# SonghuaHu-UMD/MultiSTGraph

Hardware: AMD Instinct MI355X
Metric: forward node-steps/s (B*T*N per second), MultiATGCN.predict (higher is better)
Workload: dtype f32; 1 GPU; Baltimore 403-node, in=24h out=24h, batch=64/GPU, multi+unidirection K=5; nodes=403, per_gpu_batch=64, global_batch=64, in_steps=24, out_steps=24, parallelism=batch shards, no data-path collective (dp1), layer_wavefront_streams=True

## Files before the change

multistgraph_amd/csrc/matgcn_capi.hip:

```cpp
#include <hip/hip_runtime.h>
#include <stdint.h>
#include <stdio.h>
#include <stdlib.h>
#include <string.h>

#include "../../include/matgcn.h"
#include "matgcn_internal.h"

#include "matgcn_kernels.hip"
#include "matgcn_node16.hip"
#include "matgcn_bwd_kernels.hip"
#include "matgcn_mc_scores.hip"
#include "matgcn_conformal.hip"
#include "matgcn_regions.hip"
#include "matgcn_optim.hip"
#include "matgcn_loss.hip"
#include "matgcn_region_loss.hip"
#include "matgcn_crps.hip"
#include "matgcn_head_mc_bwd.hip"

namespace {

constexpr int H = 64;
constexpr int MAX_STEPS = 64;
// ... 927 lines not shown
      CHECK_LAUNCH();
      if (multi && l + 1 < P.L) HIP_OK(hipEventRecord(W.step[l][t], cs));
      return MATGCN_OK;
    }
    if (l > 0 && t == nextChunk[l]) {
      const int nt = chunk_steps(P, t);
      nextChunk[l] = t + nt;
      float* slot; long stride;
      int mixedSteps = 0;
      if (shared_mix_slot(c, l - 1, t, &slot, &stride)) mixedSteps = P.T - 1 - t < nt ? P.T - 1 - t : nt;
      if (multi) {
        if (mixedSteps == nt) HIP_OK(hipStreamWaitEvent(xs, W.mixed[l - 1][t + nt], 0));
        else HIP_OK(hipStreamWaitEvent(xs, W.step[l - 1][t + nt - 1], 0));
      }
      RETURN_IF(hoist_x(c, l, below + t * stepRows, t, nt, xs, mixedSteps));
      if (multi) {
        HIP_OK(hipEventRecord(W.xdone[l][t], xs));
        HIP_OK(hipStreamWaitEvent(cs, W.xdone[l][t], 0));
      }
    }
    Node16Args res;
    if (l == 0)
      fill_res_args(c, l, x0p + (long)t * P.Np * P.C0, (long)P.T * P.Np * P.C0,
                    c.prm->weights_gru + (size_t)l * P.T + t, seq + t * stepRows, &res);
    else
      fill_res_args(c, l, below + t * stepRows, (long)P.Np * H, c.prm->weights_gru + (size_t)l * P.T + t,
                    seq + t * stepRows, &res);
    const bool zs = zeroStart && t == 0;
    if (!zs) RETURN_IF(cell_phase(c, l, t, 0, nullptr, &res, cs));
    if (multi && l + 1 < P.L) HIP_OK(hipEventRecord(W.mixed[l][t], cs));
    if (lazyPrep && multi && l == 0 && t == 0) RETURN_IF(prep_wait(cs, 1));
    RETURN_IF(cell_phase(c, l, t, 1, nullptr, &res, cs, zs));
    if (!zs) RETURN_IF(cell_phase(c, l, t, 2, nullptr, &res, cs));
    RETURN_IF(cell_phase(c, l, t, 3, nullptr, &res, cs, zs));
    if (multi && l + 1 < P.L) HIP_OK(hipEventRecord(W.step[l][t], cs));
    return MATGCN_OK;
  };
  for (int l = 0; l < P.L; ++l)
    for (int t = 0; t < P.T; ++t) RETURN_IF(enqueue_step(l, t));
  for (int l = 0; l < P.L; ++l) {
    hipStream_t cs = chain_stream(l);
    if (finalsUser) {
      hipLaunchKernelGGL(k_unpack_rows, dim3(blocks_for((size_t)P.B * P.N * H)), dim3(256), 0, cs, c.ws + P.oHx[l],
                         finalsUser + (size_t)l * P.B * P.N * H, P.B, P.N, P.Np, H);
      CHECK_LAUNCH();
    }
    if (multi && l > 0) HIP_OK(hipEventRecord(W.done[l], cs));
  }
  if (multi)
    for (int l = 1; l < P.L; ++l) HIP_OK(hipStreamWaitEvent(c.s, W.done[l], 0));
  return MATGCN_OK;
}

int encoder_padded(const Ctx& c, const float* x0p, const float* h0User, float* finalsUser) {
  const int rc = encoder_chains(c, x0p, h0User, finalsUser);
  if (rc != MATGCN_OK) join_library_streams(c.s);
  return rc;
}

int fuse_padded(const Ctx& c, const float* X, float* x0p, const int32_t* labelStart = nullptr,
                const int32_t* relSteps = nullptr, int64_t seriesSteps = 0) {
  const Plan& P = c.P;
  const matgcn_dims* D = c.D;
  FuseArgs a;
  memset(&a, 0, sizeof(a));
  a.X = X; a.x0 = x0p; a.tsg = c.prm->weight_tsg;
  a.labelStart = labelStart; a.seriesSteps = (long)seriesSteps;
  if (labelStart)
    for (int s2 = 0; s2 < D->x_steps; ++s2) a.rel[s2] = relSteps[s2];
  for (int h = 0; h < D->n_heads; ++h) { a.ts[h] = c.prm->weight_ts[h]; a.headBegin[h] = D->head_begin[h]; }
  for (int j = 0; j < P.C0 - P.od; ++j) a.extSrc[j] = D->ext_src[j];
  a.B = P.B; a.T = P.T; a.N = P.N; a.Np = P.Np; a.C0 = P.C0; a.od = P.od; a.F = D->x_feat;
  a.xSteps = D->x_steps; a.startDim = D->start_dim; a.nHeads = D->n_heads; a.nTs = D->n_ts;
  hipLaunchKernelGGL(k_fuse_heads, dim3(blocks_for((size_t)P.B * P.T * P.Np)), dim3(256), 0, c.s, a);
  return launch_ok();
}

int head_padded(const Ctx& c, const float* seqp, float* out) {
  const Plan& P = c.P;
  HeadArgs a;
  a.seq = seqp + (size_t)(P.T - P.headT) * P.B * P.Np * H; a.w = c.prep + P.oHead;
  a.bias = c.prm->end_conv_bias; a.out = out;
  a.B = P.B; a.T = P.headT; a.N = P.N; a.Np = P.Np; a.CH = P.CH; a.od = P.od; a.NTc = P.NTc;
  ProfScope prof(MATGCN_PROF_HEAD, c.s);
  hipLaunchKernelGGL(k_head, dim3((unsigned)(P.B * ((P.N + 31) / 32))), dim3(256), 0, c.s, a);
  return launch_ok();
}

int make_drop_desc(const matgcn_dropout* in, DropDesc* d) {
  if (!in || !d) return MATGCN_ERR_NULL;
  if (!(in->p >= 0.f && in->p < 1.f)) return MATGCN_ERR_BAD_ARG;
  memset(d, 0, sizeof(*d));
  d->seed = in->seed; d->offset = in->offset;
  d->thr = (unsigned int)((double)in->p * 4294967296.0);
  d->scale = (float)(1.0 / (1.0 - (double)in->p));
  d->on = 1;
  return MATGCN_OK;
}

int head_mc_padded(const Ctx& c, const float* seqp, const DropDesc& d, int samples, float* mean, float* stdev,
                   float* samplesOut) {
  const Plan& P = c.P;
  if (P.headT > 4 * HEAD_MC_STEPS || P.NTc > 2) return MATGCN_ERR_UNSUPPORTED;
  HeadMcArgs m;
  memset(&m, 0, sizeof(m));
  HeadArgs& a = m.h;
  a.seq = seqp + (size_t)(P.T - P.headT) * P.B * P.Np * H; a.w = c.prep + P.oHead;
  a.bias = c.prm->end_conv_bias; a.out = nullptr;
  a.B = P.B; a.T = P.headT; a.N = P.N; a.Np = P.Np; a.CH = P.CH; a.od = P.od; a.NTc = P.NTc;
  m.drop = d; m.samples = samples; m.mean = mean; m.stdev = stdev; m.samplesOut = samplesOut;
  ProfScope prof(MATGCN_PROF_HEAD, c.s);
  hipLaunchKernelGGL(k_head_mc, dim3((unsigned)(P.B * ((P.N + 31) / 32))), dim3(256), 0, c.s, m);
  return launch_ok();
}

int make_ctx(Ctx* c, const matgcn_dims* dims, const matgcn_params* params, const void* prepared, void* workspace,
             size_t workspace_bytes, void* stream, bool joinPrepare = true) {
  if (!dims || !params || !workspace) return MATGCN_ERR_NULL;
  RETURN_IF(make_plan(dims, &c->P));
  if (workspace_bytes < (size_t)c->P.workspaceFloats * sizeof(float)) return MATGCN_ERR_SMALL_BUFFER;
  c->D = dims; c->prm = params; c->prep = (const float*)prepared; c->ws = (float*)workspace;
  c->wsBytes = workspace_bytes;
  c->s = (hipStream_t)stream;
  if (prepared && joinPrepare) RETURN_IF(prep_wait(c->s, 3));
  return MATGCN_OK;
}

int check_layer_params(const matgcn_dims* D, const matgcn_params* p) {
  if (!D->gcn_off && (!p->node_emb || !p->weights_gru)) return MATGCN_ERR_NULL;
  for (int l = 0; l < D->layers; ++l) {
    if (!p->res_gate[l].weight || !p->res_gate[l].bias || !p->res_update[l].weight || !p->res_update[l].bias)
      return MATGCN_ERR_NULL;
    if (D->gcn_off) continue;
    if (!p->gate[l].weights_pool || !p->gate[l].bias_pool || !p->update[l].weights_pool || !p->update[l].bias_pool)
      return MATGCN_ERR_NULL;
    if (D->scale_by_g && (!p->gate[l].weights_g || !p->update[l].weights_g)) return MATGCN_ERR_NULL;
    if (!p->res_gate[l].weight || !p->res_gate[l].bias || !p->res_update[l].weight || !p->res_update[l].bias)
      return MATGCN_ERR_NULL;
  }
  return MATGCN_OK;
}

int stage_single_step(const Ctx& c, int layer, const float* x, const float* h, bool xpart, float** xin_out) {
  const Plan& P = c.P;
  if (layer < 0 || layer >= P.L) return MATGCN_ERR_BAD_ARG;
  if (P.gcnOff && xpart) return MATGCN_ERR_UNSUPPORTED;
  RETURN_IF(node_kernels_ready(P.nodeLds));
  float* xin = (layer == 0) ? c.ws + P.oX0p : c.ws + P.oSeq[layer - 1];
  hipLaunchKernelGGL(k_pack_rows, dim3(blocks_for((size_t)P.B * P.Np * P.Cl[layer])), dim3(256), 0, c.s, x, xin, P.B,
                     P.N, P.Np, P.Cl[layer]);
  CHECK_LAUNCH();
  hipLaunchKernelGGL(k_pack_rows, dim3(blocks_for((size_t)P.B * P.Np * H)), dim3(256), 0, c.s, h, c.ws + P.oHx[layer],
                     P.B, P.N, P.Np, H);
  CHECK_LAUNCH();
  RETURN_IF(zero_async(c.ws + P.oZHx[layer], (long)P.B * P.Np * H, c.s));
  if (xpart) {
    if (layer == 0) RETURN_IF(fold_x0(c, xin, 1, c.s));
    else RETURN_IF(hoist_x(c, layer, xin, 0, 1, c.s));
  }
  *xin_out = xin;
  return MATGCN_OK;
}

}

extern "C" {

int matgcn_abi_version(void) { return MATGCN_ABI_VERSION; }
// ... 562 lines not shown
```

multistgraph_amd/csrc/matgcn_kernels.hip:

```cpp
#include <hip/hip_runtime.h>
#include <stdint.h>

#include "matgcn_internal.h"

typedef __attribute__((ext_vector_type(16))) float f32x16;
typedef unsigned int u32x4 __attribute__((ext_vector_type(4)));
typedef __attribute__((ext_vector_type(4))) float f32x4;
#define MFMA16(a, b, c) __builtin_amdgcn_mfma_f32_16x16x4f32((a), (b), (c), 0, 0, 0)

#define MFMA32(a, b, c) __builtin_amdgcn_mfma_f32_32x32x2f32((a), (b), (c), 0, 0, 0)

__device__ __forceinline__ float sigmoid_f(float x) { return 1.0f / (1.0f + expf(-x)); }

__device__ __forceinline__ int acc_row(int r, int half) { return (r & 3) + 8 * (r >> 2) + 4 * half; }

__global__ __launch_bounds__(256) void k_adaptive_adj(const float* __restrict__ e1, const float* __restrict__ e2,
                                                      int rank, int bidir, int N, float* __restrict__ plain, int ldP) {
  extern __shared__ float logits[];
  __shared__ float red[256];
  __shared__ float erow[64];
  const int n = blockIdx.x, tid = threadIdx.x;
  for (int r = tid; r < rank; r += 256) erow[r] = e1[(size_t)n * rank + r];
  __syncthreads();
  float mx = 0.f;
// ... 601 lines not shown
__global__ __launch_bounds__(256) void k_x0_to_matrix(const float* __restrict__ x0p, float* __restrict__ X0m, int rows,
                                                      int Np, int C0, int ld) {
  const size_t idx = (size_t)blockIdx.x * 256 + threadIdx.x;
  const size_t total = (size_t)Np * ld;
  if (idx >= total) return;
  const int col = idx % ld;
  const int m = idx / ld;
  float v = 0.f;
  if (col < rows * C0) {
    const int row = col / C0, c = col - row * C0;
    v = x0p[((size_t)row * Np + m) * C0 + c];
  }
  X0m[idx] = v;
}

__global__ __launch_bounds__(256) void k_build_xa0(const float* __restrict__ X0m, const float* __restrict__ MX0,
                                                   float* __restrict__ XA0, int B, int T, int N, int Np, int C0,
                                                   int Ks, int Kx, int ld, int bChunk, int tChunk) {
  extern __shared__ float xs[];
  const int n = blockIdx.x, b0 = blockIdx.y * bChunk, t0 = blockIdx.z * tChunk;
  const int nb = min(bChunk, B - b0), nt = min(tChunk, T - t0);
  const int run = nt * C0, perK = nb * run;
  for (int i = threadIdx.x; i < (Ks + 1) * perK; i += 256) {
    const int k = i / perK, r = i - k * perK;
    const int bb = r / run, q = r - bb * run;
    const float* src = k == 0 ? X0m + (size_t)n * ld : MX0 + ((size_t)(k - 1) * Np + n) * ld;
    xs[i] = src[((size_t)(b0 + bb) * T + t0) * C0 + q];
  }
  __syncthreads();
  const int nx = (Ks + 1) * C0, kx4 = Kx >> 2, perT = nb * kx4;
  for (int i = threadIdx.x; i < nt * perT; i += 256) {
    const int tt = i / perT, r = i - tt * perT;
    const int bb = r / kx4, j0 = 4 * (r - bb * kx4);
    float v[4];
#pragma unroll
    for (int e = 0; e < 4; ++e) {
      const int j = j0 + e;
      v[e] = 0.f;
      if (j < nx) {
        const int k = j / C0, c = j - k * C0;
        v[e] = xs[(k * nb + bb) * run + tt * C0 + c];
      } else if (j == nx) v[e] = 1.0f;
    }
    float* dst = XA0 + (((size_t)(t0 + tt) * N + n) * B + b0) * Kx + 4 * (size_t)r;
    *reinterpret_cast<float4*>(dst) = make_float4(v[0], v[1], v[2], v[3]);
  }
}

struct StateInitArgs {
  float* zhx[4];
  float* hx[4];
  float* h0dst[4];
  const float* h0[4];
  float* seq[4];
};
__global__ __launch_bounds__(256) void k_state_init(StateInitArgs a, int B, int rowsSeq, int N, int Np) {
  const int l = blockIdx.y;
  const size_t idx = (size_t)blockIdx.x * 256 + threadIdx.x;
  const size_t state4 = (size_t)B * Np * 16;
  const float4 zero = make_float4(0.f, 0.f, 0.f, 0.f);
  if (idx < state4) {
    const int c4 = (int)(idx & 15);
    const int n = (int)((idx >> 4) % Np);
    const size_t r = (idx >> 4) / Np;
    float4 v = zero;
    if (a.h0[l] && n < N) {
      const float* src = a.h0[l] + (r * N + n) * 64 + 4 * c4;
      v = make_float4(src[0], src[1], src[2], src[3]);
    }
    reinterpret_cast<float4*>(a.zhx[l])[idx] = zero;
    reinterpret_cast<float4*>(a.hx[l])[idx] = v;
    if (a.h0dst[l]) reinterpret_cast<float4*>(a.h0dst[l])[idx] = v;
    return;
  }
  const int per4 = (Np - N) * 16;
  const size_t q = idx - state4;
  if (q >= (size_t)rowsSeq * per4) return;
  const size_t r = q / per4;
  const int e = (int)(q - r * per4);
  *reinterpret_cast<float4*>(a.seq[l] + (r * Np + N) * 64 + 4 * e) = zero;
}

constexpr int MIX_FLUSH_TILES = 16;

__device__ __forceinline__ void mix_tile_order(int id, int nColUnits, int nRowTiles, int& rowTile, int& colUnit) {
  if ((nColUnits & 7) == 0) {
    const int xcd = id & 7, j = id >> 3, cpx = nColUnits >> 3;
    rowTile = j % nRowTiles;
    colUnit = xcd * cpx + j / nRowTiles;
  } else {
    rowTile = id % nRowTiles;
    colUnit = id / nRowTiles;
  }
}

template <int ROLE, bool FLUSH = false>
__global__ __launch_bounds__(256) void k_mix(MixArgs a) {
  __shared__ __attribute__((aligned(16))) float As[2][16 * 64];
  __shared__ __attribute__((aligned(16))) float Bs[2][16 * 64];
  int colTile, rowTile;
  mix_tile_order(blockIdx.x, a.nColTiles, a.nRowTiles, rowTile, colTile);
  const int row0 = rowTile * 64;
  const int tid = threadIdx.x, lane = tid & 63, w = tid >> 6;
  const int wr = w >> 1, wc = w & 1, j = lane & 15, kq = lane >> 4;
  const int kk = tid >> 4, sg = tid & 15;
  const int part = blockIdx.y;
  const float* ap = a.St + (size_t)part * a.aPartStride + (size_t)kk * a.ldS + row0 + sg * 4;
  const float* bp = a.X + (size_t)part * a.xPartStride + (size_t)colTile * a.xTileStride + (size_t)kk * a.ldX + sg * 4;
  const int stPos = kk * 64 + (((sg + 4 * (kk & 3)) & 15) << 2);
  const int last = a.nK - 1;
  auto ldA = [&](int t) { return *reinterpret_cast<const float4*>(ap + (size_t)min(t, last) * 16 * a.ldS); };
  auto ldB = [&](int t) { return *reinterpret_cast<const float4*>(bp + (size_t)min(t, last) * 16 * a.ldX); };
  float4 ra0, rb0, ra1, rb1;
  {
    const float4 a0 = ldA(0), b0 = ldB(0);
    __builtin_amdgcn_sched_barrier(0);
    ra0 = ldA(1); rb0 = ldB(1); ra1 = ldA(2); rb1 = ldB(2);
    __builtin_amdgcn_sched_barrier(0);
    *reinterpret_cast<float4*>(&As[0][stPos]) = a0;
    *reinterpret_cast<float4*>(&Bs[0][stPos]) = b0;
  }
  __syncthreads();
  f32x4 acc[2][2], tot[FLUSH ? 2 : 1][2];
#pragma unroll
  for (int p = 0; p < 2; ++p)
#pragma unroll
    for (int q = 0; q < 2; ++q) {
      acc[p][q] = f32x4{0.f, 0.f, 0.f, 0.f};
      if constexpr (FLUSH) tot[p][q] = f32x4{0.f, 0.f, 0.f, 0.f};
    }
  const int rotA0 = (wr * 32 + j + 16 * kq) & 63, rotA1 = (wr * 32 + 16 + j + 16 * kq) & 63;
  const int rotB0 = (wc * 32 + j + 16 * kq) & 63, rotB1 = (wc * 32 + 16 + j + 16 * kq) & 63;
  auto mma = [&](int cur) {
    const float* A = &As[cur][kq * 64];
    const float* Bm = &Bs[cur][kq * 64];
#pragma unroll
    for (int s = 0; s < 4; ++s) {
      const float a0 = A[s * 256 + rotA0], a1 = A[s * 256 + rotA1];
      const float b0 = Bm[s * 256 + rotB0], b1 = Bm[s * 256 + rotB1];
      acc[0][0] = MFMA16(a0, b0, acc[0][0]);
      acc[0][1] = MFMA16(a0, b1, acc[0][1]);
      acc[1][0] = MFMA16(a1, b0, acc[1][0]);
      acc[1][1] = MFMA16(a1, b1, acc[1][1]);
    }
  };
  for (int it = 0; it < a.nK; it += 2) {
    mma(0);
    *reinterpret_cast<float4*>(&As[1][stPos]) = ra0;
    *reinterpret_cast<float4*>(&Bs[1][stPos]) = rb0;
    ra0 = ldA(it + 3); rb0 = ldB(it + 3);
    __syncthreads();
    if (it + 1 < a.nK) {
      mma(1);
      *reinterpret_cast<float4*>(&As[0][stPos]) = ra1;
      *reinterpret_cast<float4*>(&Bs[0][stPos]) = rb1;
      ra1 = ldA(it + 4); rb1 = ldB(it + 4);
      __syncthreads();
    }
    if constexpr (FLUSH) {
      if (((it + 2) & (MIX_FLUSH_TILES - 1)) == 0) {
#pragma unroll
        for (int p = 0; p < 2; ++p)
#pragma unroll
          for (int q = 0; q < 2; ++q) {
#pragma unroll
            for (int e = 0; e < 4; ++e) tot[p][q][e] += acc[p][q][e];
            acc[p][q] = f32x4{0.f, 0.f, 0.f, 0.f};
          }
      }
    }
  }
  if constexpr (FLUSH) {
#pragma unroll
    for (int p = 0; p < 2; ++p)
#pragma unroll
      for (int q = 0; q < 2; ++q)
#pragma unroll
        for (int e = 0; e < 4; ++e) acc[p][q][e] += tot[p][q][e];
  }
  float* stg = (w < 2 ? &As[0][0] : &Bs[0][0]) + (w & 1) * 1024;
  {
    const int jq = j >> 2, jr = j & 3, kb = kq & 1;
    int xe[4];
#pragma unroll
    for (int e = 0; e < 4; ++e) xe[e] = e * 32 + ((jq ^ e) << 2) + jr;
#pragma unroll
    for (int p = 0; p < 2; ++p)
#pragma unroll
      for (int q = 0; q < 2; ++q) {
        const int base = (p * 16 + 4 * kq) * 32 + ((q ^ kb) << 4);
#pragma unroll
        for (int e = 0; e < 4; ++e) stg[base + xe[e]] = acc[p][q][e];
      }
  }
  const bool wt = a.outFloats > 0 && a.outFloats < (1L << 29);
  float* outp = a.out + (size_t)part * a.outPartStride;
  const auto rsrc = __builtin_amdgcn_make_buffer_rsrc(outp, 0, wt ? (int)(a.outFloats * 4) : 0, 0x00020000);
  float4 v4[4];
#pragma unroll
  for (int u = 0; u < 4; ++u) {
    const int lrow = u * 8 + (lane >> 3), q = lane & 7;
    v4[u] = *reinterpret_cast<const float4*>(&stg[lrow * 32 + ((q ^ (lrow & 7)) << 2)]);
  }
#pragma unroll
  for (int u = 0; u < 4; ++u) {
    const int lrow = u * 8 + (lane >> 3), q = lane & 7;
    const float4 v = v4[u];
    const int row = row0 + wr * 32 + lrow;
    const int stride = ROLE != 2 ? a.stackStride : a.Np;
    const int k = row / stride, n = row - k * stride;
    const bool ok = k < a.Ks && n < a.N;
    const size_t off = (size_t)colTile * a.sT + (size_t)n * a.sN + (size_t)k * a.sK + wc * 32 + q * 4;
    if (wt) {
      const u32x4 bits = {__float_as_uint(v.x), __float_as_uint(v.y), __float_as_uint(v.z), __float_as_uint(v.w)};
      __builtin_amdgcn_raw_buffer_store_b128(bits, rsrc, ok ? (int)(off * 4) : (int)0x7ffffff0, 0, 16);
    } else if (ok) {
      *reinterpret_cast<float4*>(outp + off) = v;
    }
  }
}

template <int ROLE>
__global__ __launch_bounds__(256) void k_mix_c32(MixArgs a) {
  __shared__ __attribute__((aligned(16))) float As[2][16 * 64];
  __shared__ __attribute__((aligned(16))) float Bs[2][16 * 64];
  int ct2, rowTile;
  mix_tile_order(blockIdx.x, 2 * a.nColTiles, a.nRowTiles, rowTile, ct2);
  const int colTile = ct2 >> 1, half = ct2 & 1;
  const int row0 = rowTile * 64;
  const int tid = threadIdx.x, lane = tid & 63, w = tid >> 6;
  const int wr = w >> 1, wc = w & 1, j = lane & 15, kq = lane >> 4;
  const int kk = tid >> 4, sg = tid & 15, sgB = sg & 7;
  const int part = blockIdx.y;
  const float* ap = a.St + (size_t)part * a.aPartStride + (size_t)kk * a.ldS + row0 + sg * 4;
  const float* bp = a.X + (size_t)part * a.xPartStride + (size_t)colTile * a.xTileStride + (size_t)kk * a.ldX + half * 32 + sgB * 4;
  const int stPosA = kk * 64 + (((sg + 4 * (kk & 3)) & 15) << 2);
  const int stPosB = kk * 64 + (((sgB + 4 * (kk & 3)) & 15) << 2);
  const int last = a.nK - 1;
  auto ldA = [&](int t) { return *reinterpret_cast<const float4*>(ap + (size_t)min(t, last) * 16 * a.ldS); };
  auto ldB = [&](int t) { return *reinterpret_cast<const float4*>(bp + (size_t)min(t, last) * 16 * a.ldX); };
  float4 ra0, rb0, ra1, rb1;
  {
    const float4 a0 = ldA(0), b0 = ldB(0);
    __builtin_amdgcn_sched_barrier(0);
    ra0 = ldA(1); rb0 = ldB(1); ra1 = ldA(2); rb1 = ldB(2);
    __builtin_amdgcn_sched_barrier(0);
    *reinterpret_cast<float4*>(&As[0][stPosA]) = a0;
    *reinterpret_cast<float4*>(&Bs[0][stPosB]) = b0;
  }
  __syncthreads();
  f32x4 acc[2];
  acc[0] = f32x4{0.f, 0.f, 0.f, 0.f}; acc[1] = acc[0];
  const int rotA0 = (wr * 32 + j + 16 * kq) & 63, rotA1 = (wr * 32 + 16 + j + 16 * kq) & 63;
  const int rotB0 = (wc * 16 + j + 16 * kq) & 63;
  auto mma = [&](int cur) {
    const float* A = &As[cur][kq * 64];
    const float* Bm = &Bs[cur][kq * 64];
#pragma unroll
    for (int s4 = 0; s4 < 4; ++s4) {
      const float a0 = A[s4 * 256 + rotA0], a1 = A[s4 * 256 + rotA1];
      const float b0 = Bm[s4 * 256 + rotB0];
      acc[0] = MFMA16(a0, b0, acc[0]);
      acc[1] = MFMA16(a1, b0, acc[1]);
    }
  };
  for (int it = 0; it < a.nK; it += 2) {
    mma(0);
    *reinterpret_cast<float4*>(&As[1][stPosA]) = ra0;
    *reinterpret_cast<float4*>(&Bs[1][stPosB]) = rb0;
    ra0 = ldA(it + 3); rb0 = ldB(it + 3);
    __syncthreads();
    if (it + 1 < a.nK) {
      mma(1);
      *reinterpret_cast<float4*>(&As[0][stPosA]) = ra1;
      *reinterpret_cast<float4*>(&Bs[0][stPosB]) = rb1;
      ra1 = ldA(it + 4); rb1 = ldB(it + 4);
      __syncthreads();
    }
  }
  float* stg = (w < 2 ? &As[0][0] : &Bs[0][0]) + (w & 1) * 1024;
  {
    const int jq = j >> 2, jr = j & 3;
#pragma unroll
    for (int p = 0; p < 2; ++p)
#pragma unroll
      for (int e = 0; e < 4; ++e) {
        const int lrow = p * 16 + 4 * kq + e;
        stg[lrow * 16 + ((jq ^ (lrow & 3)) << 2) + jr] = acc[p][e];
      }
  }
  const bool wt = a.outFloats > 0 && a.outFloats < (1L << 29);
  float* outp = a.out + (size_t)part * a.outPartStride;
  const auto rsrc = __builtin_amdgcn_make_buffer_rsrc(outp, 0, wt ? (int)(a.outFloats * 4) : 0, 0x00020000);
  float4 v2[2];
#pragma unroll
  for (int u = 0; u < 2; ++u) {
    const int lrow = u * 16 + (lane >> 2), q = lane & 3;
    v2[u] = *reinterpret_cast<const float4*>(&stg[lrow * 16 + ((q ^ (lrow & 3)) << 2)]);
  }
#pragma unroll
  for (int u = 0; u < 2; ++u) {
    const int lrow = u * 16 + (lane >> 2), q = lane & 3;
    const float4 v = v2[u];
    const int row = row0 + wr * 32 + lrow;
    const int k = row / a.Np, n = row - k * a.Np;
    const bool ok = k < a.Ks && n < a.N;
    const size_t off = (size_t)colTile * a.sT + (size_t)n * a.sN + (size_t)k * a.sK + half * 32 + wc * 16 + q * 4;
    if (wt) {
      const u32x4 bits = {__float_as_uint(v.x), __float_as_uint(v.y), __float_as_uint(v.z), __float_as_uint(v.w)};
      __builtin_amdgcn_raw_buffer_store_b128(bits, rsrc, ok ? (int)(off * 4) : (int)0x7ffffff0, 0, 16);
    } else if (ok) {
      *reinterpret_cast<float4*>(outp + off) = v;
    }
  }
}

__device__ __forceinline__ void k_mix_n32_bf_loop(const MixArgs& a, unsigned int (*As)[16 * 32], unsigned int (*Bs)[16 * 128],
                                                  int row0, int colPair, int part, f32x4 (&acc)[2][2]);
template <bool BF = false>
__global__ __launch_bounds__(256) void k_mix_n32(MixArgs a) {
  __shared__ __attribute__((aligned(16))) float As[2][16 * 32];
  __shared__ __attribute__((aligned(16))) float Bs[2][16 * 128];
  int colPair, rowTile;
  mix_tile_order(blockIdx.x, a.nColTiles >> 1, a.nRowTiles, rowTile, colPair);
  const int row0 = rowTile * 32;
  const int tid = threadIdx.x, lane = tid & 63, w = tid >> 6;
  const int j = lane & 15, kq = lane >> 4;
  const int part = blockIdx.y;
  f32x4 acc[2][2];
  if constexpr (BF) {
    k_mix_n32_bf_loop(a, reinterpret_cast<unsigned int (*)[16 * 32]>(As), reinterpret_cast<unsigned int (*)[16 * 128]>(Bs),
                          row0, colPair, part, acc);
  } else {
  const int akk = (tid & 127) >> 3, asg = tid & 7;
  const int bkk = tid >> 4, bsg = tid & 15;
  const float* ap = a.St + (size_t)part * a.aPartStride + (size_t)akk * a.ldS + row0 + asg * 4;
  const float* bp0 = a.X + (size_t)part * a.xPartStride + (size_t)(2 * colPair) * a.xTileStride + (size_t)bkk * a.ldX + bsg * 4;
  const float* bp1 = bp0 + a.xTileStride;
  const int aPos = akk * 32 + ((asg * 4 + 16 * (akk & 1)) & 31);
  const int bPos0 = bkk * 128 + ((bsg * 4 + 16 * (bkk & 1)) & 127);
  const int bPos1 = bkk * 128 + ((64 + bsg * 4 + 16 * (bkk & 1)) & 127);
  const int last = a.nK - 1;
  auto ldA = [&](int t) { return *reinterpret_cast<const float4*>(ap + (size_t)min(t, last) * 16 * a.ldS); };
  auto ldB0 = [&](int t) { return *reinterpret_cast<const float4*>(bp0 + (size_t)min(t, last) * 16 * a.ldX); };
  auto ldB1 = [&](int t) { return *reinterpret_cast<const float4*>(bp1 + (size_t)min(t, last) * 16 * a.ldX); };
  float4 ra0, rb00, rb01, ra1, rb10, rb11;
  {
    const float4 a0 = ldA(0), b0 = ldB0(0), b1 = ldB1(0);
    __builtin_amdgcn_sched_barrier(0);
    ra0 = ldA(1); rb00 = ldB0(1); rb01 = ldB1(1); ra1 = ldA(2); rb10 = ldB0(2); rb11 = ldB1(2);
    __builtin_amdgcn_sched_barrier(0);
    *reinterpret_cast<float4*>(&As[0][aPos]) = a0;
    *reinterpret_cast<float4*>(&Bs[0][bPos0]) = b0;
    *reinterpret_cast<float4*>(&Bs[0][bPos1]) = b1;
  }
  __syncthreads();
#pragma unroll
  for (int p = 0; p < 2; ++p)
#pragma unroll
    for (int q = 0; q < 2; ++q) acc[p][q] = f32x4{0.f, 0.f, 0.f, 0.f};
  const int rot = 16 * (kq & 1);
// ... 351 lines not shown
      split_bf16x3(rb[2 * i].y, rb[2 * i + 1].y, h1[i], m1[i], l1[i]);
    }
    Bs[0][skg][bcol] = u32x4{h0[0], h0[1], h0[2], h0[3]};
    Bs[0][skg][bcol + 1] = u32x4{h1[0], h1[1], h1[2], h1[3]};
    Bs[1][skg][bcol] = u32x4{m0[0], m0[1], m0[2], m0[3]};
    Bs[1][skg][bcol + 1] = u32x4{m1[0], m1[1], m1[2], m1[3]};
    Bs[2][skg][bcol] = u32x4{l0[0], l0[1], l0[2], l0[3]};
    Bs[2][skg][bcol + 1] = u32x4{l1[0], l1[1], l1[2], l1[3]};
  };
  load(0);
  store();
  load(1);
  __syncthreads();
  f32x4 acc[2][2][2], tot[FLUSH ? 2 : 1][4];
#pragma unroll
  for (int p = 0; p < 2; ++p)
#pragma unroll
    for (int q = 0; q < 4; ++q) {
      acc[q >> 1][p][q & 1] = f32x4{0.f, 0.f, 0.f, 0.f};
      if constexpr (FLUSH) tot[p][q] = f32x4{0.f, 0.f, 0.f, 0.f};
    }
  auto fragA = [&](int piece, int p) { return __builtin_bit_cast(bf16x8v_t, As[piece][kq][wr * 32 + p * 16 + j]); };
  auto fragB = [&](int piece, int q) { return __builtin_bit_cast(bf16x8v_t, Bs[piece][kq][wc * 64 + q * 16 + j]); };
  auto mma = [&]() {
    bf16x8v_t fa[3][2];
#pragma unroll
    for (int piece = 0; piece < 3; ++piece)
#pragma unroll
      for (int p = 0; p < 2; ++p) fa[piece][p] = fragA(piece, p);
#pragma unroll
    for (int q = 0; q < 4; ++q) {
      const bf16x8v_t bh = fragB(0, q), bm = fragB(1, q), bl = fragB(2, q);
#pragma unroll
      for (int p = 0; p < 2; ++p) acc[q >> 1][p][q & 1] = __builtin_amdgcn_mfma_f32_16x16x32_bf16(fa[0][p], bl, acc[q >> 1][p][q & 1], 0, 0, 0);
#pragma unroll
      for (int p = 0; p < 2; ++p) acc[q >> 1][p][q & 1] = __builtin_amdgcn_mfma_f32_16x16x32_bf16(fa[2][p], bh, acc[q >> 1][p][q & 1], 0, 0, 0);
#pragma unroll
      for (int p = 0; p < 2; ++p) acc[q >> 1][p][q & 1] = __builtin_amdgcn_mfma_f32_16x16x32_bf16(fa[1][p], bm, acc[q >> 1][p][q & 1], 0, 0, 0);
#pragma unroll
      for (int p = 0; p < 2; ++p) acc[q >> 1][p][q & 1] = __builtin_amdgcn_mfma_f32_16x16x32_bf16(fa[0][p], bm, acc[q >> 1][p][q & 1], 0, 0, 0);
#pragma unroll
      for (int p = 0; p < 2; ++p) acc[q >> 1][p][q & 1] = __builtin_amdgcn_mfma_f32_16x16x32_bf16(fa[1][p], bh, acc[q >> 1][p][q & 1], 0, 0, 0);
#pragma unroll
      for (int p = 0; p < 2; ++p) acc[q >> 1][p][q & 1] = __builtin_amdgcn_mfma_f32_16x16x32_bf16(fa[0][p], bh, acc[q >> 1][p][q & 1], 0, 0, 0);
    }
  };
  for (int t = 0; t < nTot; ++t) {
    mma();
    __syncthreads();
    if (t + 1 < nTot) {
      store();
      load(t + 2);
    }
    __syncthreads();
    if constexpr (FLUSH) {
      if (((t + 1) & (MIX_FLUSH_TILES / 2 - 1)) == 0) {
#pragma unroll
        for (int p = 0; p < 2; ++p)
#pragma unroll
          for (int q = 0; q < 4; ++q) {
#pragma unroll
            for (int e = 0; e < 4; ++e) tot[p][q][e] += acc[q >> 1][p][q & 1][e];
            acc[q >> 1][p][q & 1] = f32x4{0.f, 0.f, 0.f, 0.f};
          }
      }
    }
  }
  if constexpr (FLUSH) {
#pragma unroll
    for (int p = 0; p < 2; ++p)
#pragma unroll
      for (int q = 0; q < 4; ++q)
#pragma unroll
        for (int e = 0; e < 4; ++e) acc[q >> 1][p][q & 1][e] += tot[p][q][e];
  }
  const int colTile = 2 * colPair + wc;
  if (colTile < a.nColTiles) {
    float* stg = reinterpret_cast<float*>(&Bs[0][0][0]) + w * 1024;
#pragma unroll
    for (int half = 0; half < 2; ++half) mix_store_tile(a, part, stg, acc[half], row0 + wr * 32, colTile, half * 32);
  }
}

__global__ __launch_bounds__(256) void k_head(HeadArgs a) {
  __shared__ f32x16 part[3][2][64];
  const int tilesPerB = (a.N + 31) >> 5;
  const int b = blockIdx.x / tilesPerB, n0 = (blockIdx.x % tilesPerB) * 32;
  const int lane = threadIdx.x & 63, w = threadIdx.x >> 6, i = lane & 31, half = lane >> 5;
  const int node = min(n0 + i, a.Np - 1);
  f32x16 acc[2];
#pragma unroll
  for (int tt = 0; tt < 2; ++tt)
#pragma unroll
    for (int r = 0; r < 16; ++r) acc[tt][r] = 0.f;
  const int nt = a.NTc;
  for (int t = w; t < a.T; t += 4) {
    const float* rowp = a.seq + (((size_t)t * a.B + b) * a.Np + node) * 64 + half * 4;
#pragma unroll
    for (int g = 0; g < 8; ++g) {
      const float4 a4 = *reinterpret_cast<const float4*>(rowp + g * 8);
      const int jg = t * 8 + g;
      for (int tt = 0; tt < nt; ++tt) {
        const float4 w4 = *reinterpret_cast<const float4*>(a.w + ((size_t)(jg * nt + tt) * 64 + lane) * 4);
        acc[tt] = MFMA32(a4.x, w4.x, acc[tt]);
        acc[tt] = MFMA32(a4.y, w4.y, acc[tt]);
        acc[tt] = MFMA32(a4.z, w4.z, acc[tt]);
        acc[tt] = MFMA32(a4.w, w4.w, acc[tt]);
      }
    }
  }
  if (w > 0) { part[w - 1][0][lane] = acc[0]; part[w - 1][1][lane] = acc[1]; }
  __syncthreads();
  if (w > 0) return;
#pragma unroll
  for (int q = 0; q < 3; ++q) {
    const f32x16 p0 = part[q][0][lane], p1 = part[q][1][lane];
#pragma unroll
    for (int r = 0; r < 16; ++r) { acc[0][r] += p0[r]; acc[1][r] += p1[r]; }
  }
  for (int tt = 0; tt < nt; ++tt) {
    const int ch = tt * 32 + i;
    if (ch >= a.CH) continue;
    const float bias = a.bias[ch];
    const int o = ch / a.od, dd = ch - o * a.od;
#pragma unroll
    for (int r = 0; r < 16; ++r) {
      const int n = n0 + acc_row(r, half);
      if (n < a.N) a.out[(((size_t)b * (a.CH / a.od) + o) * a.N + n) * a.od + dd] = acc[tt][r] + bias;
    }
  }
}

constexpr int HEAD_MC_STEPS = 6;
template <int K> struct HeadStep { static constexpr int value = K; };
__global__ __launch_bounds__(256) void k_head_mc(HeadMcArgs m) {
  const HeadArgs& a = m.h;
  __shared__ f32x16 part[3][2][64];
  __shared__ float stat[2][32][64];
  const int tilesPerB = (a.N + 31) >> 5;
  const int b = blockIdx.x / tilesPerB, n0 = (blockIdx.x % tilesPerB) * 32;
  const int lane = threadIdx.x & 63, w = __builtin_amdgcn_readfirstlane(threadIdx.x >> 6), i = lane & 31, half = lane >> 5;
  const int node = min(n0 + i, a.Np - 1);
  const int nt = a.NTc;
  float4 av[HEAD_MC_STEPS][8];
#pragma unroll
  for (int k = 0; k < HEAD_MC_STEPS; ++k) {
    const int t = w + 4 * k;
    const float* rowp = a.seq + (((size_t)min(t, a.T - 1) * a.B + b) * a.Np + node) * 64 + half * 4;
#pragma unroll
    for (int g = 0; g < 8; ++g) av[k][g] = *reinterpret_cast<const float4*>(rowp + g * 8);
  }
  float bias[2];
#pragma unroll
  for (int tt = 0; tt < 2; ++tt) bias[tt] = (tt < nt && tt * 32 + i < a.CH) ? a.bias[tt * 32 + i] : 0.f;
  if (w == 0) {
#pragma unroll
    for (int e = 0; e < 32; ++e) { stat[0][e][lane] = 0.f; stat[1][e][lane] = 0.f; }
  }
  const size_t sampleFloats = (size_t)a.B * a.CH * a.N;
  const int tFirst = min(w, a.T - 1);
  auto wload = [&](const float* wbase, int jg, float4 (&dst)[2]) __attribute__((always_inline)) {
#pragma unroll
    for (int tt = 0; tt < 2; ++tt)
      dst[tt] = *reinterpret_cast<const float4*>(wbase + ((size_t)(jg * nt + min(tt, nt - 1)) * 64 + lane) * 4);
  };
  float4 wc[2];
  wload(a.w, tFirst * 8, wc);
  const unsigned long long qLane = ((unsigned long long)b * a.T * a.N + (n0 + i)) * 16 + half;
  for (int s = 0; s < m.samples; ++s) {
    DropDesc d = m.drop;
    d.offset += (unsigned long long)s;
    const float* wbase = a.w;
    asm volatile("" : "+s"(wbase));
    unsigned int qlo = (unsigned int)qLane, qhi = (unsigned int)(qLane >> 32);
    asm volatile("" : "+v"(qlo), "+v"(qhi));
    const unsigned long long qb = ((unsigned long long)qhi << 32) | qlo;
    f32x16 acc[2];
#pragma unroll
    for (int tt = 0; tt < 2; ++tt)
#pragma unroll
      for (int r = 0; r < 16; ++r) acc[tt][r] = 0.f;
    auto step = [&](auto kc) __attribute__((always_inline)) {
      constexpr int k = decltype(kc)::value;
      const int t = w + 4 * k;
      if (t < a.T) {
        const unsigned long long q0 = qb + (unsigned long long)t * a.N * 16;
        const int tNext = t + 4 < a.T ? t + 4 : tFirst;
#pragma unroll
        for (int g = 0; g < 8; ++g) {
          float4 wn[2];
          wload(wbase, (g < 7 ? t : tNext) * 8 + ((g + 1) & 7), wn);
          const float4 mk = drop_mult4(d, q0 + 2 * g);
          const float4 a4 = make_float4(av[k][g].x * mk.x, av[k][g].y * mk.y, av[k][g].z * mk.z, av[k][g].w * mk.w);
#pragma unroll
          for (int tt = 0; tt < 2; ++tt) {
            if (tt < nt) {
              acc[tt] = MFMA32(a4.x, wc[tt].x, acc[tt]);
              acc[tt] = MFMA32(a4.y, wc[tt].y, acc[tt]);
              acc[tt] = MFMA32(a4.z, wc[tt].z, acc[tt]);
              acc[tt] = MFMA32(a4.w, wc[tt].w, acc[tt]);
            }
          }
          wc[0] = wn[0]; wc[1] = wn[1];
// ... 258 lines not shown
```

Before: 98.14 million node-steps/s.

## Software-pipeline head kernel loads and tighten mix K-loop scheduling

The head kernel is templated on the channel tile count and now prefetches the next timestep's activations and weights into registers while the current step's MFMAs run. The previous version issued dependent loads inside the MFMA loop. The mix kernels' K loops are restructured into full pairs plus an odd tail, with sched_barrier hints placed between the LDS stores and the next global loads, and a register-clobber hint is added. The cost is higher register pressure, which could lower occupancy, and a new unsupported-config check for NTc outside 1..2.

```diff
diff --git a/multistgraph_amd/csrc/matgcn_capi.hip b/multistgraph_amd/csrc/matgcn_capi.hip
--- a/multistgraph_amd/csrc/matgcn_capi.hip
+++ b/multistgraph_amd/csrc/matgcn_capi.hip
@@ -1033,8 +1033,9 @@
   a.seq = seqp + (size_t)(P.T - P.headT) * P.B * P.Np * H; a.w = c.prep + P.oHead;
   a.bias = c.prm->end_conv_bias; a.out = out;
   a.B = P.B; a.T = P.headT; a.N = P.N; a.Np = P.Np; a.CH = P.CH; a.od = P.od; a.NTc = P.NTc;
+  if (P.NTc < 1 || P.NTc > 2) return MATGCN_ERR_UNSUPPORTED;
   ProfScope prof(MATGCN_PROF_HEAD, c.s);
-  hipLaunchKernelGGL(k_head, dim3((unsigned)(P.B * ((P.N + 31) / 32))), dim3(256), 0, c.s, a);
+  hipLaunchKernelGGL(P.NTc == 1 ? k_head<1> : k_head<2>, dim3((unsigned)(P.B * ((P.N + 31) / 32))), dim3(256), 0, c.s, a);
   return launch_ok();
 }
 
diff --git a/multistgraph_amd/csrc/matgcn_kernels.hip b/multistgraph_amd/csrc/matgcn_kernels.hip
--- a/multistgraph_amd/csrc/matgcn_kernels.hip
+++ b/multistgraph_amd/csrc/matgcn_kernels.hip
@@ -707,6 +707,7 @@
 }
 
 constexpr int MIX_FLUSH_TILES = 16;
+#define MIX_STAGE_ORDER() __builtin_amdgcn_sched_barrier(0x10E)
 
 __device__ __forceinline__ void mix_tile_order(int id, int nColUnits, int nRowTiles, int& rowTile, int& colUnit) {
   if ((nColUnits & 7) == 0) {
@@ -723,6 +724,7 @@
 __global__ __launch_bounds__(256) void k_mix(MixArgs a) {
   __shared__ __attribute__((aligned(16))) float As[2][16 * 64];
   __shared__ __attribute__((aligned(16))) float Bs[2][16 * 64];
+  if constexpr (!FLUSH) asm volatile("" ::: "v55", "a23");
   int colTile, rowTile;
   mix_tile_order(blockIdx.x, a.nColTiles, a.nRowTiles, rowTile, colTile);
   const int row0 = rowTile * 64;
@@ -769,21 +771,9 @@
       acc[1][1] = MFMA16(a1, b1, acc[1][1]);
     }
   };
-  for (int it = 0; it < a.nK; it += 2) {
-    mma(0);
-    *reinterpret_cast<float4*>(&As[1][stPos]) = ra0;
-    *reinterpret_cast<float4*>(&Bs[1][stPos]) = rb0;
-    ra0 = ldA(it + 3); rb0 = ldB(it + 3);
-    __syncthreads();
-    if (it + 1 < a.nK) {
-      mma(1);
-      *reinterpret_cast<float4*>(&As[0][stPos]) = ra1;
-      *reinterpret_cast<float4*>(&Bs[0][stPos]) = rb1;
-      ra1 = ldA(it + 4); rb1 = ldB(it + 4);
-      __syncthreads();
-    }
+  auto flush = [&](int done) {
     if constexpr (FLUSH) {
-      if (((it + 2) & (MIX_FLUSH_TILES - 1)) == 0) {
+      if ((done & (MIX_FLUSH_TILES - 1)) == 0) {
 #pragma unroll
         for (int p = 0; p < 2; ++p)
 #pragma unroll
@@ -794,6 +784,28 @@
           }
       }
     }
+  };
+  const int nPairs = a.nK >> 1;
+  for (int pr = 0; pr < nPairs; ++pr) {
+    const int it = 2 * pr;
+    mma(0);
+    *reinterpret_cast<float4*>(&As[1][stPos]) = ra0;
+    *reinterpret_cast<float4*>(&Bs[1][stPos]) = rb0;
+    MIX_STAGE_ORDER();
+    ra0 = ldA(it + 3); rb0 = ldB(it + 3);
+    __syncthreads();
+    mma(1);
+    *reinterpret_cast<float4*>(&As[0][stPos]) = ra1;
+    *reinterpret_cast<float4*>(&Bs[0][stPos]) = rb1;
+    MIX_STAGE_ORDER();
+    ra1 = ldA(it + 4); rb1 = ldB(it + 4);
+    __syncthreads();
+    flush(it + 2);
+  }
+  if (a.nK & 1) {
+    mma(0);
+    __syncthreads();
+    flush(a.nK + 1);
   }
   if constexpr (FLUSH) {
 #pragma unroll
@@ -889,19 +901,25 @@
       acc[1] = MFMA16(a1, b0, acc[1]);
     }
   };
-  for (int it = 0; it < a.nK; it += 2) {
+  const int nPairs = a.nK >> 1;
+  for (int pr = 0; pr < nPairs; ++pr) {
+    const int it = 2 * pr;
     mma(0);
     *reinterpret_cast<float4*>(&As[1][stPosA]) = ra0;
     *reinterpret_cast<float4*>(&Bs[1][stPosB]) = rb0;
+    MIX_STAGE_ORDER();
     ra0 = ldA(it + 3); rb0 = ldB(it + 3);
     __syncthreads();
-    if (it + 1 < a.nK) {
-      mma(1);
-      *reinterpret_cast<float4*>(&As[0][stPosA]) = ra1;
-      *reinterpret_cast<float4*>(&Bs[0][stPosB]) = rb1;
-      ra1 = ldA(it + 4); rb1 = ldB(it + 4);
-      __syncthreads();
-    }
+    mma(1);
+    *reinterpret_cast<float4*>(&As[0][stPosA]) = ra1;
+    *reinterpret_cast<float4*>(&Bs[0][stPosB]) = rb1;
+    MIX_STAGE_ORDER();
+    ra1 = ldA(it + 4); rb1 = ldB(it + 4);
+    __syncthreads();
+  }
+  if (a.nK & 1) {
+    mma(0);
+    __syncthreads();
   }
   float* stg = (w < 2 ? &As[0][0] : &Bs[0][0]) + (w & 1) * 1024;
   {
@@ -1419,43 +1437,77 @@
   }
 }
 
+template <int NT, bool MORE>
+__device__ __forceinline__ void head_step(f32x16 (&acc)[NT], float4 (&av)[8], float4 (&wv)[8][NT],
+                                          const float* __restrict__ rowpNext, const float* __restrict__ wNext) {
+#pragma unroll
+  for (int g = 0; g < 8; ++g) {
+#pragma unroll
+    for (int tt = 0; tt < NT; ++tt) {
+      acc[tt] = MFMA32(av[g].x, wv[g][tt].x, acc[tt]);
+      acc[tt] = MFMA32(av[g].y, wv[g][tt].y, acc[tt]);
+      acc[tt] = MFMA32(av[g].z, wv[g][tt].z, acc[tt]);
+      acc[tt] = MFMA32(av[g].w, wv[g][tt].w, acc[tt]);
+    }
+    if constexpr (MORE) {
+      av[g] = *reinterpret_cast<const float4*>(rowpNext + g * 8);
+#pragma unroll
+      for (int tt = 0; tt < NT; ++tt)
+        wv[g][tt] = *reinterpret_cast<const float4*>(wNext + (size_t)((g * NT + tt) * 64) * 4);
+    }
+    __builtin_amdgcn_sched_barrier(0);
+  }
+}
+
+template <int NT>
 __global__ __launch_bounds__(256) void k_head(HeadArgs a) {
-  __shared__ f32x16 part[3][2][64];
+  __shared__ f32x16 part[3][NT][64];
   const int tilesPerB = (a.N + 31) >> 5;
   const int b = blockIdx.x / tilesPerB, n0 = (blockIdx.x % tilesPerB) * 32;
-  const int lane = threadIdx.x & 63, w = threadIdx.x >> 6, i = lane & 31, half = lane >> 5;
+  const int lane = threadIdx.x & 63, w = __builtin_amdgcn_readfirstlane(threadIdx.x >> 6), i = lane & 31, half = lane >> 5;
   const int node = min(n0 + i, a.Np - 1);
-  f32x16 acc[2];
-#pragma unroll
-  for (int tt = 0; tt < 2; ++tt)
+  f32x16 acc[NT];
+#pragma unroll
+  for (int tt = 0; tt < NT; ++tt)
 #pragma unroll
     for (int r = 0; r < 16; ++r) acc[tt][r] = 0.f;
-  const int nt = a.NTc;
-  for (int t = w; t < a.T; t += 4) {
-    const float* rowp = a.seq + (((size_t)t * a.B + b) * a.Np + node) * 64 + half * 4;
+  if (w < a.T) {
+    const size_t stepFloats = (size_t)a.B * a.Np * 64;
+    const float* rowp = a.seq + ((size_t)w * a.B + b) * a.Np * 64 + (size_t)node * 64 + half * 4;
+    const float* wp = a.w + ((size_t)w * 8 * NT * 64 + lane) * 4;
+    float4 av[8], wv[8][NT];
 #pragma unroll
     for (int g = 0; g < 8; ++g) {
-      const float4 a4 = *reinterpret_cast<const float4*>(rowp + g * 8);
-      const int jg = t * 8 + g;
-      for (int tt = 0; tt < nt; ++tt) {
-        const float4 w4 = *reinterpret_cast<const float4*>(a.w + ((size_t)(jg * nt + tt) * 64 + lane) * 4);
-        acc[tt] = MFMA32(a4.x, w4.x, acc[tt]);
-        acc[tt] = MFMA32(a4.y, w4.y, acc[tt]);
-        acc[tt] = MFMA32(a4.z, w4.z, acc[tt]);
-        acc[tt] = MFMA32(a4.w, w4.w, acc[tt]);
-      }
-    }
-  }
-  if (w > 0) { part[w - 1][0][lane] = acc[0]; part[w - 1][1][lane] = acc[1]; }
+      av[g] = *reinterpret_cast<const float4*>(rowp + g * 8);
+#pragma unroll
+      for (int tt = 0; tt < NT; ++tt) wv[g][tt] = *reinterpret_cast<const float4*>(wp + (size_t)((g * NT + tt) * 64) * 4);
+      __builtin_amdgcn_sched_barrier(0);
+    }
+    int t = w;
+    for (; t + 4 < a.T; t += 4) {
+      rowp += 4 * stepFloats;
+      wp += (size_t)4 * 8 * NT * 64 * 4;
+      head_step<NT, true>(acc, av, wv, rowp, wp);
+    }
+    head_step<NT, false>(acc, av, wv, nullptr, nullptr);
+  }
+  if (w > 0) {
+#pragma unroll
+    for (int tt = 0; tt < NT; ++tt) part[w - 1][tt][lane] = acc[tt];
+  }
   __syncthreads();
   if (w > 0) return;
 #pragma unroll
   for (int q = 0; q < 3; ++q) {
-    const f32x16 p0 = part[q][0][lane], p1 = part[q][1][lane];
-#pragma unroll
-    for (int r = 0; r < 16; ++r) { acc[0][r] += p0[r]; acc[1][r] += p1[r]; }
-  }
-  for (int tt = 0; tt < nt; ++tt) {
+#pragma unroll
+    for (int tt = 0; tt < NT; ++tt) {
+      const f32x16 p = part[q][tt][lane];
+#pragma unroll
+      for (int r = 0; r < 16; ++r) acc[tt][r] += p[r];
+    }
+  }
+#pragma unroll
+  for (int tt = 0; tt < NT; ++tt) {
     const int ch = tt * 32 + i;
     if (ch >= a.CH) continue;
     const float bias = a.bias[ch];
```

Measured after the change: 98.70 million node-steps/s, median of 6. Within noise of the previous version (+0.6%).
